# wizyoung/YOLOv3_TensorFlow

Measured on NVIDIA H100. Metric: images/sec, higher is better.
Workload: dtype f16

## Files before the change

yolov3_tensorflow_b200/csrc/common.cuh:

```cuda
#pragma once
#include <cuda.h>
#include <cuda_runtime.h>
#include <cuda_fp16.h>
#include <cuda_bf16.h>
#include <cuda_fp8.h>
#include <stdint.h>
#include <stdio.h>

#include "../../include/yolob200.h"

namespace yb {

void set_error(const char* fmt, ...);
int cuda_fail(cudaError_t e, const char* what, const char* file, int line);

#define YB_CUDA(call)                                                        \
  do {                                                                       \
    cudaError_t _e = (call);                                                 \
    if (_e != cudaSuccess) return yb::cuda_fail(_e, #call, __FILE__, __LINE__); \
  } while (0)

#define YB_REQUIRE(cond, ...)                \
  do {                                       \
    if (!(cond)) {                           \
// ... 105 lines not shown
}
__device__ __forceinline__ void mbar_wait(uint64_t* bar, uint32_t parity) {
  uint32_t spins = 0;
  while (!mbar_try_wait(bar, parity)) {
    if (++spins > (1u << 26)) __trap();
  }
}

__device__ __forceinline__ void tma_prefetch_desc(const CUtensorMap* m) {
  asm volatile("prefetch.tensormap [%0];" ::"l"(reinterpret_cast<uint64_t>(m)) : "memory");
}
__device__ __forceinline__ void tma_load_2d(void* dst, const CUtensorMap* m, uint64_t* bar, int c0, int c1) {
  asm volatile(
      "cp.async.bulk.tensor.2d.shared::cluster.global.tile.mbarrier::complete_tx::bytes [%0], [%1, {%3, %4}], [%2];"
      ::"r"(smem_u32(dst)), "l"(reinterpret_cast<uint64_t>(m)), "r"(smem_u32(bar)), "r"(c0), "r"(c1)
      : "memory");
}
__device__ __forceinline__ void tma_load_im2col_4d(void* dst, const CUtensorMap* m, uint64_t* bar, int c, int w,
                                                   int h, int n, uint16_t ow, uint16_t oh) {
  asm volatile(
      "cp.async.bulk.tensor.4d.shared::cluster.global.im2col.mbarrier::complete_tx::bytes"
      " [%0], [%1, {%3, %4, %5, %6}], [%2], {%7, %8};"
      ::"r"(smem_u32(dst)), "l"(reinterpret_cast<uint64_t>(m)), "r"(smem_u32(bar)), "r"(c), "r"(w), "r"(h),
      "r"(n), "h"(ow), "h"(oh)
      : "memory");
}

__device__ __forceinline__ void tma_store_2d(const CUtensorMap* m, const void* src, int c0, int c1) {
  asm volatile("cp.async.bulk.tensor.2d.global.shared::cta.bulk_group [%0, {%2, %3}], [%1];" ::"l"(
                   reinterpret_cast<uint64_t>(m)),
               "r"(smem_u32(src)), "r"(c0), "r"(c1)
               : "memory");
}
__device__ __forceinline__ void bulk_commit_group() { asm volatile("cp.async.bulk.commit_group;" ::: "memory"); }
template <int N>
__device__ __forceinline__ void bulk_wait_group_read() {
  asm volatile("cp.async.bulk.wait_group.read %0;" ::"n"(N) : "memory");
}
template <int N>
__device__ __forceinline__ void bulk_wait_group() {
  asm volatile("cp.async.bulk.wait_group %0;" ::"n"(N) : "memory");
}

__device__ __forceinline__ void stmatrix_x4(uint32_t saddr, uint32_t r0, uint32_t r1, uint32_t r2, uint32_t r3) {
  asm volatile("stmatrix.sync.aligned.m8n8.x4.shared.b16 [%0], {%1, %2, %3, %4};" ::"r"(saddr), "r"(r0), "r"(r1), "r"(r2),
               "r"(r3)
               : "memory");
}
__device__ __forceinline__ void ldmatrix_x4(uint32_t saddr, uint32_t& r0, uint32_t& r1, uint32_t& r2, uint32_t& r3) {
  asm volatile("ldmatrix.sync.aligned.m8n8.x4.shared.b16 {%0, %1, %2, %3}, [%4];"
               : "=r"(r0), "=r"(r1), "=r"(r2), "=r"(r3)
               : "r"(saddr)
               : "memory");
}

__device__ __forceinline__ uint32_t cluster_ctarank() {
  uint32_t r;
  asm volatile("mov.u32 %0, %%cluster_ctarank;" : "=r"(r));
  return r;
}
__device__ __forceinline__ void cluster_sync_all() {
  __syncwarp();
  asm volatile("barrier.cluster.arrive.release.aligned;" ::: "memory");
  asm volatile("barrier.cluster.wait.acquire.aligned;" ::: "memory");
}
__device__ __forceinline__ void mbar_arrive_remote(uint64_t* bar, uint32_t cta) {
// ... 58 lines not shown
```

yolov3_tensorflow_b200/csrc/conv.cuh:

```cuda
#pragma once
#include "common.cuh"
#include "decode.cuh"

namespace yb {

struct ConvParams {
  int M, P, Q;
  int cout;
  int cin;
  int ksize, stride, pad;
  int kh, kw;
  int scatter;
  int im2col;
  int consumers;
  int cluster;
  int cluster_n;
  int epi_reg;
  int pingpong;
  int ctas;
  int num_m_tiles, num_n_tiles;
  const float* scale;
  const float* shift;
  void* out;
  long out_ld;
// ... 7 lines not shown
  int res_smem;
  CUtensorMap tmR;
  int epi_tma;
  CUtensorMap tmO;
  int dtype;
  int block_n;
  int block_kb;
  int det_e;
};

struct ConvLaunch {
  CUtensorMap tmA, tmB;
  ConvParams p;
};

struct ConvRequest {
  yb_conv_desc d;
  int kh = 0, kw = 0, scatter = 0;
  bool stats = false;
  bool res = false;
  int det_e = 0;
  bool plan_rule = false;
};

int conv_select(const ConvRequest& r, ConvParams* p);
int conv_prepare(const ConvRequest& r, const void* x, const void* w_packed, const float* scale, const float* shift,
                 const void* res, void* out, float* stat_sum, float* stat_sqsum, ConvLaunch* l);
inline size_t dgrad_s2_class_offset(int c, int cin_pad, int k_cout) {
  static constexpr int first[4] = {0, 1, 3, 5};
  return (size_t)first[c] * cin_pad * k_cout;
}
int conv_prepare_dgrad_s2(const yb_conv_desc* fwd, const void* dz, int dz_ld, int k_cout, const void* w_dgrad_s2,
                          const void* res, int res_ld, void* dx, int dx_ld, ConvLaunch* l);
struct HaloMaps { CUtensorMap plane[4]; CUtensorMap w; CUtensorMap in3d; CUtensorMap res; };
struct HaloParams {
  int n, ho, wo;
  int tiles_x, tiles_y, num_tiles;
  int cout;
  int leaky;
  const float* scale;
  const float* shift;
  const void* res;
  long res_ld;
  void* out;
  long out_ld;
  const float* stem_w;
  const float* stem_scale;
  const float* stem_shift;
  int in_h, in_w;
  int out_e4m3;
  float out_inv_scale;
  int res_smem;
  int dtype;
  int cin, stride;
  int stem;
};
struct HaloRequest {
  yb_conv_desc d;
  bool res = false;
  bool out_e4m3 = false;
  bool stem = false;
};
struct HaloLaunch {
  HaloMaps maps;
  HaloParams p;
};
int halo_select(const HaloRequest& r, HaloParams* p);
// ... 33 lines not shown
```

yolov3_tensorflow_b200/csrc/conv_halo.cu:

```cuda
#include <cudaTypedefs.h>
#include <string.h>

#include <type_traits>

#include "common.cuh"
#include "conv.cuh"
#include "wgmma.cuh"

namespace yb {

int make_tmap_2d(CUtensorMap* tm, const void* base, int dtype, long rows, long cols, long ld, int box_rows, int box_cols,
                 int weights);
int make_tmap_image3d(CUtensorMap* tm, const float* base, int n, int h, int w, int box_f, int box_h);
int make_tmap_tiled4d(CUtensorMap* tm, const void* base, int dtype, int n, int h, int w, int c, long ld, int box_c,
                      int box_w, int box_h, int estride);

static constexpr int HT_H = 16, HT_W = 8;
static constexpr int HALO_THREADS = 384;
static constexpr int HALO_EPI_LD = 33;

template <int CIN, int COUT, int STRIDE, bool RES = false>
struct HaloCfg {
  static constexpr int ROWB = CIN * 2;
  static constexpr int NPLANE = STRIDE == 1 ? 1 : 4;
  static constexpr int ph(int p) { return STRIDE == 1 ? HT_H + 2 : ((p >> 1) == 0 ? HT_H + 1 : HT_H); }
  static constexpr int pw(int p) { return STRIDE == 1 ? HT_W + 2 : ((p & 1) == 0 ? HT_W + 1 : HT_W); }
  static constexpr int pbytes(int p) { return (ph(p) * pw(p) * ROWB + 1023) / 1024 * 1024; }
  static constexpr int poff(int p) { return p == 0 ? 0 : poff(p - 1) + pbytes(p - 1); }
  static constexpr int RES_OFF = poff(NPLANE - 1) + pbytes(NPLANE - 1);
  static constexpr int RES_BYTES = RES ? HT_H * HT_W * COUT * 2 : 0;
  static constexpr int STAGE_BYTES = RES_OFF + RES_BYTES;
  static constexpr int STAGE_TX = (STRIDE == 1 ? ph(0) * pw(0) * ROWB
                                               : (ph(0) * pw(0) + ph(1) * pw(1) + ph(2) * pw(2) + ph(3) * pw(3)) * ROWB) +
                                  RES_BYTES;
  static constexpr int B_TAP_BYTES = COUT * ROWB;
  static constexpr int B_BYTES = 9 * B_TAP_BYTES;
  static constexpr int EPI_BYTES = 2 * 64 * HALO_EPI_LD * 4;
  static constexpr int MISC_BYTES = 1024;
  static constexpr int BUDGET = 227 * 1024 - 1024 ;
  static constexpr int NST_RAW = (BUDGET - B_BYTES - EPI_BYTES - MISC_BYTES - 2 * COUT * 4) / STAGE_BYTES;
  static constexpr int NST = NST_RAW > 6 ? 6 : NST_RAW;
  static_assert(NST >= 1, "halo conv: configuration does not fit shared memory");
  static constexpr int SMEM_BYTES = 1024 + B_BYTES + NST * STAGE_BYTES + EPI_BYTES + MISC_BYTES + 2 * COUT * 4;
  static constexpr uint32_t SWIZZLE = ROWB;
  static constexpr int tap_plane(int r, int s) { return STRIDE == 1 ? 0 : (((r == 1) ? 2 : 0) | ((s == 1) ? 1 : 0)); }
  static constexpr int tap_dr(int r) { return STRIDE == 1 ? r : (r == 2 ? 1 : 0); }
  static constexpr int tap_ds(int s) { return STRIDE == 1 ? s : (s == 2 ? 1 : 0); }
};

struct StemCfg {
  static constexpr int SH = 2 * HT_H + 1, SW = 2 * HT_W + 1;
  static constexpr int NPX = SH * SW;
  static constexpr int NT16 = (NPX + 15) / 16;
  static constexpr int IN_ROWS = SH + 2;
  static constexpr int IN_ROWF = 60;
  static constexpr int IN_BYTES = (IN_ROWS * IN_ROWF * 4 + 127) / 128 * 128;
  static constexpr int NIN = 2;
};

__device__ __forceinline__ void tma_load_3d(void* dst, const CUtensorMap* m, uint64_t* bar, int c0, int c1, int c2) {
  asm volatile(
      "cp.async.bulk.tensor.3d.shared::cluster.global.tile.mbarrier::complete_tx::bytes [%0], [%1, {%3, %4, %5}], [%2];"
      ::"r"(smem_u32(dst)), "l"(reinterpret_cast<uint64_t>(m)), "r"(smem_u32(bar)), "r"(c0), "r"(c1), "r"(c2)
      : "memory");
}
__device__ __forceinline__ void mma16816_f16(float (&c)[4], const uint32_t (&a)[4], uint32_t b0, uint32_t b1, bool bf16) {
  if (bf16)
    asm volatile("mma.sync.aligned.m16n8k16.row.col.f32.bf16.bf16.f32 {%0,%1,%2,%3}, {%4,%5,%6,%7}, {%8,%9}, {%0,%1,%2,%3};"
                 : "+f"(c[0]), "+f"(c[1]), "+f"(c[2]), "+f"(c[3]) : "r"(a[0]), "r"(a[1]), "r"(a[2]), "r"(a[3]), "r"(b0), "r"(b1));
  else
    asm volatile("mma.sync.aligned.m16n8k16.row.col.f32.f16.f16.f32 {%0,%1,%2,%3}, {%4,%5,%6,%7}, {%8,%9}, {%0,%1,%2,%3};"
                 : "+f"(c[0]), "+f"(c[1]), "+f"(c[2]), "+f"(c[3]) : "r"(a[0]), "r"(a[1]), "r"(a[2]), "r"(a[3]), "r"(b0), "r"(b1));
}

__device__ __forceinline__ void tma_load_4d(void* dst, const CUtensorMap* m, uint64_t* bar, int c0, int c1, int c2, int c3) {
  asm volatile(
      "cp.async.bulk.tensor.4d.shared::cluster.global.tile.mbarrier::complete_tx::bytes [%0], [%1, {%3, %4, %5, %6}], [%2];"
      ::"r"(smem_u32(dst)), "l"(reinterpret_cast<uint64_t>(m)), "r"(smem_u32(bar)), "r"(c0), "r"(c1), "r"(c2), "r"(c3)
      : "memory");
}

template <typename T, int CIN, int COUT, int STRIDE, int STEMW = 0, typename TO = T, bool RES = false>
__global__ void __launch_bounds__(HALO_THREADS + 32 * STEMW, 1)
conv_halo_kernel(const __grid_constant__ HaloMaps maps, const __grid_constant__ HaloParams p) {
  using C = HaloCfg<CIN, COUT, STRIDE, RES>;
  static_assert(!RES || (CIN == 32 && COUT == 64 && STRIDE == 1 && STEMW == 0), "the residual box is Conv_3's");
  constexpr int PROD_WARP0 = HALO_THREADS / 32;
  static_assert(STEMW == 0 || (CIN == 32 && STRIDE == 2), "the fused stem feeds Conv_1 (32 -> 64, stride 2)");
  extern __shared__ uint8_t smem_raw[];
  uint8_t* smem = smem_raw + ((1024u - (smem_u32(smem_raw) & 1023u)) & 1023u);
  uint8_t* sB = smem;
  uint8_t* sA = smem + C::B_BYTES;
  float* sE = reinterpret_cast<float*>(sA + C::NST * C::STAGE_BYTES);
  uint64_t* bars = reinterpret_cast<uint64_t*>(reinterpret_cast<uint8_t*>(sE) + C::EPI_BYTES);
  uint64_t* full_bar = bars;
  uint64_t* empty_bar = bars + 8;
  uint64_t* b_bar = bars + 20;
  float* s_ss = reinterpret_cast<float*>(reinterpret_cast<uint8_t*>(sE) + C::EPI_BYTES + C::MISC_BYTES);
  uint64_t* in_full = bars + 24;
  uint64_t* in_empty = bars + 26;
  uint8_t* sIn = reinterpret_cast<uint8_t*>(s_ss + 2 * COUT);

  const int warp = threadIdx.x >> 5, lane = threadIdx.x & 31;

  if (warp == 0 && lane == 0) {
    if (STEMW == 0) {
#pragma unroll
      for (int i = 0; i < C::NPLANE; ++i) tma_prefetch_desc(&maps.plane[i]);
    }
    tma_prefetch_desc(&maps.w);
    if (RES) tma_prefetch_desc(&maps.res);
    for (int i = 0; i < C::NST; ++i) { mbar_init(&full_bar[i], STEMW > 0 ? STEMW : 1); mbar_init(&empty_bar[i], 8); }
    if (STEMW > 0) {
      tma_prefetch_desc(&maps.in3d);
      for (int i = 0; i < StemCfg::NIN; ++i) { mbar_init(&in_full[i], 1); mbar_init(&in_empty[i], STEMW); }
    }
    mbar_init(b_bar, 1);
    fence_barrier_init();
  }
  for (int c = threadIdx.x; c < COUT; c += blockDim.x) {
    s_ss[c] = c < p.cout ? __ldg(p.scale + c) : 0.f;
    s_ss[COUT + c] = c < p.cout ? __ldg(p.shift + c) : 0.f;
  }
  __syncthreads();

  if (warp == 0) {
    if (lane == 0) {
      mbar_arrive_expect_tx(b_bar, (uint32_t)C::B_BYTES);
#pragma unroll
      for (int t = 0; t < 9; ++t) tma_load_2d(sB + t * C::B_TAP_BYTES, &maps.w, b_bar, t * CIN, 0);
      int stage = 0;
      uint32_t phase = 0;
      if (STEMW > 0) {
        for (int tile = blockIdx.x; tile < p.num_tiles; tile += gridDim.x) {
          const int tx = tile % p.tiles_x;
          const int ty = (tile / p.tiles_x) % p.tiles_y;
          const int img = tile / (p.tiles_x * p.tiles_y);
          mbar_wait(&in_empty[stage], phase ^ 1);
          mbar_arrive_expect_tx(&in_full[stage], (uint32_t)(StemCfg::IN_ROWS * StemCfg::IN_ROWF * 4));
          tma_load_3d(sIn + stage * StemCfg::IN_BYTES, &maps.in3d, &in_full[stage], (2 * tx * HT_W - 2) * 3 - 2, 2 * ty * HT_H - 2, img);
          if (++stage == StemCfg::NIN) { stage = 0; phase ^= 1; }
        }
      }
      for (int tile = blockIdx.x; STEMW == 0 && tile < p.num_tiles; tile += gridDim.x) {
        const int tx = tile % p.tiles_x;
        const int ty = (tile / p.tiles_x) % p.tiles_y;
        const int img = tile / (p.tiles_x * p.tiles_y);
        const int h0 = ty * HT_H, w0 = tx * HT_W;
        mbar_wait(&empty_bar[stage], phase ^ 1);
        mbar_arrive_expect_tx(&full_bar[stage], (uint32_t)C::STAGE_TX);
        uint8_t* dst = sA + stage * C::STAGE_BYTES;
        if (STRIDE == 1) {
          tma_load_4d(dst, &maps.plane[0], &full_bar[stage], 0, w0 - 1, h0 - 1, img);
          if (RES) tma_load_4d(dst + C::RES_OFF, &maps.res, &full_bar[stage], 0, w0, h0, img);
        } else {
#pragma unroll
          for (int pl = 0; pl < 4; ++pl) {
            const int hs = 2 * h0 - ((pl >> 1) == 0 ? 1 : 0), ws = 2 * w0 - ((pl & 1) == 0 ? 1 : 0);
            tma_load_4d(dst + C::poff(pl), &maps.plane[pl], &full_bar[stage], 0, ws, hs, img);
          }
        }
        if (++stage == C::NST) { stage = 0; phase ^= 1; }
      }
    }
  } else if (warp >= 4 && warp < PROD_WARP0) {
    constexpr bool kBF16 = std::is_same<T, __nv_bfloat16>::value;
    const int cw = (warp - 4) >> 2;
    const int t = threadIdx.x & 127;
    const int bar_id = 1 + cw;
    float* stg = sE + cw * 64 * HALO_EPI_LD;
    const bool has_res = STEMW == 0 && p.res != nullptr;
    const int er = t >> 1, eh = t & 1;
    const uint32_t a_base = smem_u32(sA), b_base = smem_u32(sB);
    float acc[COUT / 2];
    mbar_wait(b_bar, 0);
    int stage = 0;
    uint32_t phase = 0;
    for (int tile = blockIdx.x; tile < p.num_tiles; tile += gridDim.x) {
      mbar_wait(&full_bar[stage], phase);
      const uint32_t st_base = a_base + stage * C::STAGE_BYTES;
      wgmma_fence_operand(acc);
      wgmma_fence();
#pragma unroll
      for (int r = 0; r < 3; ++r) {
#pragma unroll
        for (int s = 0; s < 3; ++s) {
          const int pl = C::tap_plane(r, s);
          const uint32_t a_tap = st_base + C::poff(pl) + ((8 * cw + C::tap_dr(r)) * C::pw(pl) + C::tap_ds(s)) * C::ROWB;
          const uint32_t b_tap = b_base + (r * 3 + s) * C::B_TAP_BYTES;
#pragma unroll
          for (int k = 0; k < CIN / 16; ++k)
            Wgmma<COUT, kBF16, 0, 0>::mma(acc, make_kmajor_desc(a_tap + k * 32, C::pw(pl) * C::ROWB, C::SWIZZLE),
                                          make_kmajor_desc(b_tap + k * 32, 8 * C::ROWB, C::SWIZZLE), (r | s | k) != 0);
        }
      }
      wgmma_commit();
      wgmma_fence_operand(acc);
      wgmma_wait<0>();
      wgmma_fence_operand(acc);
      const uint8_t* sres = sA + stage * C::STAGE_BYTES + C::RES_OFF;
      const int rel_stage = stage;
      if (!RES) {
        __syncwarp();
        if (lane == 0) mbar_arrive(&empty_bar[stage]);
      }
      if (++stage == C::NST) { stage = 0; phase ^= 1; }

      const int tx = tile % p.tiles_x;
      const int ty = (tile / p.tiles_x) % p.tiles_y;
      const int img = tile / (p.tiles_x * p.tiles_y);
      const int oh = ty * HT_H + 8 * cw + (er >> 3), ow = tx * HT_W + (er & 7);
      const bool ok = oh < p.ho && ow < p.wo;
      const long off = ((long)img * p.ho + oh) * p.wo + ow;
#pragma unroll 1
      for (int ch = 0; ch < COUT / 32; ++ch) {
        warpgroup_bar(bar_id);
        wgmma_stage_chunk<COUT>(acc, ch, stg, HALO_EPI_LD, t);
        warpgroup_bar(bar_id);
        if (!ok) continue;
        const int c0 = ch * 32 + eh * 16;
        const float* src = stg + er * HALO_EPI_LD + eh * 16;
        float v[16];
#pragma unroll
        for (int j = 0; j < 16; ++j) v[j] = fmaf(src[j], s_ss[c0 + j], s_ss[COUT + c0 + j]);
        if (p.leaky) {
#pragma unroll
          for (int j = 0; j < 16; ++j) v[j] = fmaxf(v[j], 0.1f * v[j]);
        }
        if (has_res) {
          const uint4* rp = reinterpret_cast<const uint4*>(static_cast<const T*>(p.res) + off * p.res_ld + c0);
          const int px = 64 * cw + er;
          const uint8_t* rrow = sres + px * 128;
#pragma unroll
          for (int j = 0; j < 2; ++j) {
            const uint4 u = RES ? *reinterpret_cast<const uint4*>(rrow + ((((c0 >> 3) + j) ^ (px & 7)) << 4)) : __ldg(rp + j);
            float2 f;
            f = Pack2<T>::unpack(u.x); v[8 * j + 0] += f.x; v[8 * j + 1] += f.y;
            f = Pack2<T>::unpack(u.y); v[8 * j + 2] += f.x; v[8 * j + 3] += f.y;
            f = Pack2<T>::unpack(u.z); v[8 * j + 4] += f.x; v[8 * j + 5] += f.y;
            f = Pack2<T>::unpack(u.w); v[8 * j + 6] += f.x; v[8 * j + 7] += f.y;
          }
        }
        if constexpr (std::is_same<TO, __nv_fp8_e4m3>::value) {
          *reinterpret_cast<uint4*>(static_cast<uint8_t*>(p.out) + off * p.out_ld + c0) = e4m3x16_pack(v, p.out_inv_scale);
          continue;
        }
        uint4* op = reinterpret_cast<uint4*>(static_cast<T*>(p.out) + off * p.out_ld + c0);
#pragma unroll
        for (int j = 0; j < 2; ++j) {
          uint4 pk;
          pk.x = Pack2<T>::pack(v[8 * j + 0], v[8 * j + 1]);
          pk.y = Pack2<T>::pack(v[8 * j + 2], v[8 * j + 3]);
          pk.z = Pack2<T>::pack(v[8 * j + 4], v[8 * j + 5]);
          pk.w = Pack2<T>::pack(v[8 * j + 6], v[8 * j + 7]);
          op[j] = pk;
        }
      }
      if (RES) {
        __syncwarp();
        if (lane == 0) mbar_arrive(&empty_bar[rel_stage]);
      }
    }
  } else if (STEMW > 0 && warp >= PROD_WARP0) {
    const int pw_id = warp - PROD_WARP0;
    const bool bf16 = std::is_same<T, __nv_bfloat16>::value;
    const int g = lane >> 2, q = lane & 3;
    uint32_t bfrag[4][2][2];
#pragma unroll
    for (int nt = 0; nt < 4; ++nt)
#pragma unroll
      for (int ks = 0; ks < 2; ++ks)
#pragma unroll
        for (int hb = 0; hb < 2; ++hb) {
          const int n = nt * 8 + g, k = ks * 16 + hb * 8 + 2 * q;
          const float w0 = k < 27 ? __ldg(p.stem_w + n * 27 + k) : 0.f;
          const float w1 = k + 1 < 27 ? __ldg(p.stem_w + n * 27 + k + 1) : 0.f;
          bfrag[nt][ks][hb] = Pack2<T>::pack(w0, w1);
        }
    float sc[4][2], sh[4][2];
#pragma unroll
    for (int nt = 0; nt < 4; ++nt)
#pragma unroll
      for (int j = 0; j < 2; ++j) {
        sc[nt][j] = __ldg(p.stem_scale + nt * 8 + 2 * q + j);
        sh[nt][j] = __ldg(p.stem_shift + nt * 8 + 2 * q + j);
      }
    int koff[2][2][2];
#pragma unroll
    for (int ks = 0; ks < 2; ++ks)
#pragma unroll
      for (int hb = 0; hb < 2; ++hb)
#pragma unroll
        for (int j = 0; j < 2; ++j) {
          const int k = ks * 16 + hb * 8 + 2 * q + j;
// ... 53 lines not shown
      auto store = [&](const M16& m) {
#pragma unroll
        for (int hr = 0; hr < 2; ++hr) {
          if (!m.live[hr]) continue;
          uint8_t* row = planes + m.poff + m.rho[hr] * 64 + q * 4;
          const int swz = (m.rho[hr] >> 1) & 3;
          if (m.inside[hr]) {
#pragma unroll
            for (int nt = 0; nt < 4; ++nt) {
              float v0 = fmaf(m.acc[nt][2 * hr], sc[nt][0], sh[nt][0]);
              float v1 = fmaf(m.acc[nt][2 * hr + 1], sc[nt][1], sh[nt][1]);
              v0 = fmaxf(v0, 0.1f * v0); v1 = fmaxf(v1, 0.1f * v1);
              *reinterpret_cast<uint32_t*>(row + ((nt ^ swz) << 4)) = Pack2<T>::pack(v0, v1);
            }
          } else {
#pragma unroll
            for (int nt = 0; nt < 4; ++nt) *reinterpret_cast<uint32_t*>(row + ((nt ^ swz) << 4)) = 0u;
          }
        }
      };
#pragma unroll 1
      for (int t = pw_id; t < StemCfg::NT16; t += STEMW) {
        M16 m0;
        gather(t, m0);
        multiply(m0);
        store(m0);
      }
      fence_proxy_async();
      __syncwarp();
      if (lane == 0) {
        mbar_arrive(&full_bar[stage]);
        mbar_arrive(&in_empty[in_stage]);
      }
      if (++in_stage == StemCfg::NIN) { in_stage = 0; in_phase ^= 1; }
      if (++stage == C::NST) { stage = 0; phase ^= 1; }
    }
  }
}

static constexpr int STEM_WARPS = 8;

template <typename T, int CIN, int COUT, int STRIDE, int STEMW = 0, typename TO = T, bool RES = false>
struct HaloKernel {
  static constexpr int THREADS = HALO_THREADS + 32 * STEMW;
  static constexpr int SMEM_BYTES =
      HaloCfg<CIN, COUT, STRIDE, RES>::SMEM_BYTES + (STEMW > 0 ? StemCfg::NIN * StemCfg::IN_BYTES : 0);
  static_assert(SMEM_BYTES <= 227 * 1024, "halo conv: configuration does not fit shared memory");
  static constexpr auto kernel = conv_halo_kernel<T, CIN, COUT, STRIDE, STEMW, TO, RES>;
};

static int no_halo_kernel(const HaloParams& p) {
  set_error("conv_halo: no kernel for dtype %d, cin=%d cout=%d stride=%d, fused stem %d, e4m3 output %d, residual box %d",
            p.dtype, p.cin, p.cout, p.stride, p.stem, p.out_e4m3, p.res_smem);
  return YB_ERR_UNSUPPORTED;
}

template <typename T, typename F>
static int halo_kernel_type(const HaloParams& p, F& f) {
  const int ci = p.cin, co = p.cout, s = p.stride;
  if (p.stem) {
    if (ci == 32 && co == 64 && s == 2 && !p.out_e4m3 && !p.res_smem) return f(HaloKernel<T, 32, 64, 2, STEM_WARPS>());
    return no_halo_kernel(p);
  }
  if (ci == 32 && co == 64 && s == 1) {
    if (!p.out_e4m3) return p.res_smem ? f(HaloKernel<T, 32, 64, 1, 0, T, true>()) : f(HaloKernel<T, 32, 64, 1>());
    if constexpr (std::is_same<T, __half>::value)
      return p.res_smem ? f(HaloKernel<T, 32, 64, 1, 0, __nv_fp8_e4m3, true>()) : f(HaloKernel<T, 32, 64, 1, 0, __nv_fp8_e4m3>());
    return no_halo_kernel(p);
  }
  if (p.out_e4m3 || p.res_smem) return no_halo_kernel(p);
  if (ci == 32 && co == 64 && s == 2) return f(HaloKernel<T, 32, 64, 2>());
  if (ci == 32 && co == 128 && s == 1) return f(HaloKernel<T, 32, 128, 1>());
  if (ci == 32 && co == 128 && s == 2) return f(HaloKernel<T, 32, 128, 2>());
  if (ci == 64 && co == 64 && s == 1) return f(HaloKernel<T, 64, 64, 1>());
  if (ci == 64 && co == 64 && s == 2) return f(HaloKernel<T, 64, 64, 2>());
  if (ci == 64 && co == 128 && s == 1) return f(HaloKernel<T, 64, 128, 1>());
  return no_halo_kernel(p);
}

// ... 45 lines not shown
  p->out_e4m3 = r.out_e4m3;
  p->res_smem = (r.res && !r.stem && d->cin == 32 && d->cout == 64 && d->stride == 1 &&
                 strcmp(opt("YB_CONV_RES"), "ldg") != 0) ? 1 : 0;
  p->dtype = d->dtype; p->cin = d->cin; p->stride = d->stride; p->stem = r.stem;
  return halo_kernel_for(*p, [](auto) -> int { return YB_OK; });
}

bool conv_halo_supported(const yb_conv_desc* d) {
  HaloParams p;
  return halo_select(HaloRequest{*d}, &p) == YB_OK;
}

int conv_halo_prepare(const HaloRequest& r, const void* x, const void* w_packed, const float* scale, const float* shift,
                      const void* res, void* out, const float* stem_w, const float* stem_scale, const float* stem_shift,
                      HaloLaunch* l) {
  HaloParams* p = &l->p;
  HaloMaps* maps = &l->maps;
  int rc = halo_select(r, p);
  if (rc) return rc;
  const yb_conv_desc* d = &r.d;
  YB_REQUIRE(x && w_packed && scale && shift && out, "conv_halo: null pointer");
  YB_REQUIRE(r.stem ? stem_w && stem_scale && stem_shift : !stem_w && !stem_scale && !stem_shift,
             "conv_halo: the stem's weights, scale and shift are given exactly when the request fuses the stem");
  YB_REQUIRE((res != nullptr) == r.res, "conv_halo: a residual pointer is given exactly when the request has a residual");
  YB_REQUIRE(((uintptr_t)x & 15) == 0 && ((uintptr_t)w_packed & 15) == 0 && ((uintptr_t)out & 15) == 0 && ((uintptr_t)res & 15) == 0,
             "conv_halo: pointers must be 16-byte aligned");
  memset(maps, 0, sizeof(*maps));
  p->scale = scale; p->shift = shift; p->res = res; p->out = out;
  p->stem_w = stem_w; p->stem_scale = stem_scale; p->stem_shift = stem_shift;
  if (p->res_smem) {
    rc = make_tmap_tiled4d(&maps->res, res, d->dtype, d->n, p->ho, p->wo, d->cout, d->res_ld, 64, HT_W, HT_H, 1);
    if (rc) return rc;
  }
  if (r.stem) {
    rc = make_tmap_image3d(&maps->in3d, static_cast<const float*>(x), d->n, d->h, d->w, StemCfg::IN_ROWF, StemCfg::IN_ROWS);
    if (rc) return rc;
  } else if (d->stride == 1) {
    rc = make_tmap_tiled4d(&maps->plane[0], x, d->dtype, d->n, d->h, d->w, d->cin, d->in_ld, d->cin, HT_W + 2, HT_H + 2, 1);
    if (rc) return rc;
  } else {
    for (int pl = 0; pl < 4; ++pl) {
      const int rows = (pl >> 1) == 0 ? HT_H + 1 : HT_H, cols = (pl & 1) == 0 ? HT_W + 1 : HT_W;
      rc = make_tmap_tiled4d(&maps->plane[pl], x, d->dtype, d->n, d->h, d->w, d->cin, d->in_ld, d->cin, 2 * cols - 1,
                             2 * rows - 1, 2);
      if (rc) return rc;
    }
  }
  const long K = 9L * d->cin;
  return make_tmap_2d(&maps->w, w_packed, d->dtype, yb_conv_cout_pad(d->cout), K, K, d->cout, d->cin, 1);
}

}

using namespace yb;

extern "C" int yb_conv3x3_halo_supported(const yb_conv_desc* d) { return d && conv_halo_supported(d) ? 1 : 0; }

extern "C" int yb_conv3x3_halo_fwd(const yb_conv_desc* d, const void* x, const void* w_packed, const float* scale,
                                   const float* shift, const void* res, void* out, void* stream) {
  if (!d) { set_error("conv_halo: null descriptor"); return YB_ERR_INVALID_ARGUMENT; }
  HaloRequest r{*d};
  r.res = res != nullptr;
  HaloLaunch l;
  int rc = conv_halo_prepare(r, x, w_packed, scale, shift, res, out, nullptr, nullptr, nullptr, &l);
  if (rc) return rc;
  return conv_halo_launch(l, static_cast<cudaStream_t>(stream));
// ... 14 lines not shown
```

yolov3_tensorflow_b200/csrc/conv_igemm.cu:

```cuda
#include <cudaTypedefs.h>
#include <math.h>
#include <stdlib.h>
#include <string.h>

#include <type_traits>

#include "common.cuh"
#include "conv.cuh"
#include "wgmma.cuh"

namespace yb {

static constexpr int WG_ROWS = 64;
static constexpr int RING_BYTES = 196 * 1024;
static constexpr int EPI_LD = 33;
static constexpr int EPI_FLOATS = WG_ROWS * EPI_LD;

template <int BN, int BKB, int NC, bool RES = false>
struct Cfg {
  static constexpr int BLOCK_M = WG_ROWS * NC;
  static constexpr int THREADS = 128 * (NC + 1);
  static constexpr int A_BYTES = BLOCK_M * BKB;
  static constexpr int B_BYTES = BN * BKB;
  static constexpr int STAGE_BYTES = A_BYTES + B_BYTES;
// ... 222 lines not shown
        }
      } else if (cany) {
        bool pass = false;
        float sc = 0.f;
        if (cok && v >= d.logit_lo) {
          sc = __fmul_rn(cconf, sigmoid_ref(v));
          pass = sc >= d.thr;
        }
        const unsigned m = __ballot_sync(0xffffffffu, pass);
        if (m != 0u) {
          const int c = e - 5;
          const unsigned mine = m & same;
          const int leader = pass ? __ffs(mine) - 1 : lane;
          int base = 0;
          if (pass && lane == leader) base = atomicAdd(d.cand_count + img * d.C + c, __popc(mine));
          base = __shfl_sync(0xffffffffu, base, leader);
          if (pass) {
            const long seg = ((long)img * d.C + c) * d.B;
            const int slot = base + __popc(mine & lt);
            d.cand_score[seg + slot] = sc;
            d.cand_idx[seg + slot] = box0 + a;
          }
        }
      }
      if (++e == E) { e = 0; ++a; }
    }
  }
}

template <typename T, int BN, int NH, bool RES>
__device__ __forceinline__ void epilogue_tma(const ConvParams& p, const float (&acc)[NH][BN / 2], const int row0,
                                             const int n0, const float4* ss4, uint8_t* slab, const uint32_t slab_h,
                                             const uint32_t slab_b, const int lane) {
  const int r = lane & 7, mi = lane >> 3;
  const uint32_t lane_off = (uint32_t)((r + 8 * (mi & 1)) * 128 + (((mi >> 1) ^ r) << 4));
  const float slope = p.leaky ? 0.1f : 1.f;
#pragma unroll
  for (int h = 0; h < NH; ++h) {
#pragma unroll
    for (int b = 0; b < BN / 64; ++b) {
      uint8_t* s = slab + h * slab_h + b * slab_b;
      const uint32_t sa = smem_u32(s) + lane_off;
      uint32_t pk[16];
#pragma unroll
      for (int q = 0; q < 4; ++q) {
        if constexpr (RES) ldmatrix_x4(sa ^ (q << 5), pk[4 * q], pk[4 * q + 1], pk[4 * q + 2], pk[4 * q + 3]);
#pragma unroll
        for (int ih = 0; ih < 2; ++ih) {
          const int j = 8 * b + 2 * q + ih;
          const float4 c = ss4[4 * j + (lane & 3)];
#pragma unroll
          for (int hh = 0; hh < 2; ++hh) {
            float v0 = fmaf(acc[h][4 * j + 2 * hh], c.x, c.z);
            float v1 = fmaf(acc[h][4 * j + 2 * hh + 1], c.y, c.w);
            v0 = fmaxf(v0, slope * v0);
            v1 = fmaxf(v1, slope * v1);
            uint32_t& w = pk[4 * q + 2 * ih + hh];
            if constexpr (RES) {
              const float2 f = Pack2<T>::unpack(w);
              v0 += f.x; v1 += f.y;
            }
            w = Pack2<T>::pack(v0, v1);
          }
        }
        if constexpr (RES) stmatrix_x4(sa ^ (q << 5), pk[4 * q], pk[4 * q + 1], pk[4 * q + 2], pk[4 * q + 3]);
      }
      if constexpr (!RES) {
        if (lane == 0) bulk_wait_group_read<0>();
        __syncwarp();
#pragma unroll
        for (int q = 0; q < 4; ++q) stmatrix_x4(sa ^ (q << 5), pk[4 * q], pk[4 * q + 1], pk[4 * q + 2], pk[4 * q + 3]);
      }
      fence_proxy_async();
      __syncwarp();
      if (lane == 0 && row0 + h * WG_ROWS < p.M && n0 + b * 64 < p.cout) {
        tma_store_2d(&p.tmO, s, n0 + b * 64, row0 + h * WG_ROWS);
        bulk_commit_group();
      }
    }
  }
}

static constexpr int MMA_TURN_BAR = 3;

template <typename T, int BN, int BKB, int NC, int DET_E = 0, bool PP = false, int CM = 0, int CN = 1, bool RES = false,
          bool TMA = false>
__global__ void __launch_bounds__(128 * (NC + 1), 1)
conv_igemm_kernel(const __grid_constant__ CUtensorMap tmA, const __grid_constant__ CUtensorMap tmB,
                  const __grid_constant__ ConvParams p) {
  static_assert(!PP || (NC == 2 && DET_E == 0), "ping-pong: two consumer warpgroups, no fused decode");
  static_assert(!RES || (PP && sizeof(T) == 2), "the shared-memory shortcut tile is a 16-bit ping-pong variant");
  static_assert(CM != 0 || CN == 1, "a run-time cluster shape is p.cluster x 1");
  static_assert(!TMA || (sizeof(T) == 2 && NC == 2 && DET_E == 0), "the TMA-store epilogue: 16-bit, 128-row tiles, no fused decode");
  constexpr int NH = PP ? 2 : 1;
  using C = Cfg<BN, BKB, NC, RES>;
  constexpr int BK = BKB / (int)sizeof(T);
  extern __shared__ uint8_t smem_raw[];
  uint8_t* smem = smem_raw + ((1024u - (smem_u32(smem_raw) & 1023u)) & 1023u);
  uint8_t* sA = smem;
  uint8_t* sB = smem + C::STAGES * C::A_BYTES;
  uint8_t* sR = smem + C::STAGES * C::STAGE_BYTES;
  float* s_epi = reinterpret_cast<float*>(sR + C::RES_BYTES);
  float* s_stat = s_epi + NC * EPI_FLOATS;
  float* s_ss = s_stat + NC * 2 * BN;
  uint64_t* full_bar = reinterpret_cast<uint64_t*>(s_ss + NC * 2 * BN);
  uint64_t* empty_bar = full_bar + 8;
  uint64_t* res_full = empty_bar + 8;
// ... 774 lines not shown
```

yolov3_tensorflow_b200/csrc/wgmma.cuh:

```cuda
#pragma once
#include <stdint.h>

namespace yb {

template <int N, bool BF16, int TA, int TB>
struct Wgmma;

template <int TA, int TB>
struct Wgmma<32, false, TA, TB> {
  static __device__ __forceinline__ void mma(float (&d)[16], uint64_t da, uint64_t db, int scale_d) {
    asm volatile(
        "{\n.reg .pred p;\nsetp.ne.b32 p, %18, 0;\n"
        "wgmma.mma_async.sync.aligned.m64n32k16.f32.f16.f16 {%0, %1, %2, %3, %4, %5, %6, %7, %8, %9, %10, %11, %12, %13, %14, %15}, %16, %17, p, 1, 1, %19, %20;\n}\n"
        : "+f"(d[0]), "+f"(d[1]), "+f"(d[2]), "+f"(d[3]), "+f"(d[4]), "+f"(d[5]), "+f"(d[6]), "+f"(d[7]), "+f"(d[8]), "+f"(d[9]), "+f"(d[10]), "+f"(d[11]), "+f"(d[12]), "+f"(d[13]), "+f"(d[14]), "+f"(d[15])
        : "l"(da), "l"(db), "r"(scale_d), "n"(TA), "n"(TB));
  }
};

template <int TA, int TB>
struct Wgmma<32, true, TA, TB> {
  static __device__ __forceinline__ void mma(float (&d)[16], uint64_t da, uint64_t db, int scale_d) {
    asm volatile(
        "{\n.reg .pred p;\nsetp.ne.b32 p, %18, 0;\n"
        "wgmma.mma_async.sync.aligned.m64n32k16.f32.bf16.bf16 {%0, %1, %2, %3, %4, %5, %6, %7, %8, %9, %10, %11, %12, %13, %14, %15}, %16, %17, p, 1, 1, %19, %20;\n}\n"
// ... 89 lines not shown
        "{\n.reg .pred p;\nsetp.ne.b32 p, %66, 0;\n"
        "wgmma.mma_async.sync.aligned.m64n128k32.f32.e4m3.e4m3 {%0, %1, %2, %3, %4, %5, %6, %7, %8, %9, %10, %11, %12, %13, %14, %15, %16, %17, %18, %19, %20, %21, %22, %23, %24, %25, %26, %27, %28, %29, %30, %31, %32, %33, %34, %35, %36, %37, %38, %39, %40, %41, %42, %43, %44, %45, %46, %47, %48, %49, %50, %51, %52, %53, %54, %55, %56, %57, %58, %59, %60, %61, %62, %63}, %64, %65, p, 1, 1;\n}\n"
        : "+f"(d[0]), "+f"(d[1]), "+f"(d[2]), "+f"(d[3]), "+f"(d[4]), "+f"(d[5]), "+f"(d[6]), "+f"(d[7]), "+f"(d[8]), "+f"(d[9]), "+f"(d[10]), "+f"(d[11]), "+f"(d[12]), "+f"(d[13]), "+f"(d[14]), "+f"(d[15]), "+f"(d[16]), "+f"(d[17]), "+f"(d[18]), "+f"(d[19]), "+f"(d[20]), "+f"(d[21]), "+f"(d[22]), "+f"(d[23]), "+f"(d[24]), "+f"(d[25]), "+f"(d[26]), "+f"(d[27]), "+f"(d[28]), "+f"(d[29]), "+f"(d[30]), "+f"(d[31]), "+f"(d[32]), "+f"(d[33]), "+f"(d[34]), "+f"(d[35]), "+f"(d[36]), "+f"(d[37]), "+f"(d[38]), "+f"(d[39]), "+f"(d[40]), "+f"(d[41]), "+f"(d[42]), "+f"(d[43]), "+f"(d[44]), "+f"(d[45]), "+f"(d[46]), "+f"(d[47]), "+f"(d[48]), "+f"(d[49]), "+f"(d[50]), "+f"(d[51]), "+f"(d[52]), "+f"(d[53]), "+f"(d[54]), "+f"(d[55]), "+f"(d[56]), "+f"(d[57]), "+f"(d[58]), "+f"(d[59]), "+f"(d[60]), "+f"(d[61]), "+f"(d[62]), "+f"(d[63])
        : "l"(da), "l"(db), "r"(scale_d));
  }
};

template <>
struct WgmmaE4M3<256> {
  static __device__ __forceinline__ void mma(float (&d)[128], uint64_t da, uint64_t db, int scale_d) {
    asm volatile(
        "{\n.reg .pred p;\nsetp.ne.b32 p, %130, 0;\n"
        "wgmma.mma_async.sync.aligned.m64n256k32.f32.e4m3.e4m3 {%0, %1, %2, %3, %4, %5, %6, %7, %8, %9, %10, %11, %12, %13, %14, %15, %16, %17, %18, %19, %20, %21, %22, %23, %24, %25, %26, %27, %28, %29, %30, %31, %32, %33, %34, %35, %36, %37, %38, %39, %40, %41, %42, %43, %44, %45, %46, %47, %48, %49, %50, %51, %52, %53, %54, %55, %56, %57, %58, %59, %60, %61, %62, %63, %64, %65, %66, %67, %68, %69, %70, %71, %72, %73, %74, %75, %76, %77, %78, %79, %80, %81, %82, %83, %84, %85, %86, %87, %88, %89, %90, %91, %92, %93, %94, %95, %96, %97, %98, %99, %100, %101, %102, %103, %104, %105, %106, %107, %108, %109, %110, %111, %112, %113, %114, %115, %116, %117, %118, %119, %120, %121, %122, %123, %124, %125, %126, %127}, %128, %129, p, 1, 1;\n}\n"
        : "+f"(d[0]), "+f"(d[1]), "+f"(d[2]), "+f"(d[3]), "+f"(d[4]), "+f"(d[5]), "+f"(d[6]), "+f"(d[7]), "+f"(d[8]), "+f"(d[9]), "+f"(d[10]), "+f"(d[11]), "+f"(d[12]), "+f"(d[13]), "+f"(d[14]), "+f"(d[15]), "+f"(d[16]), "+f"(d[17]), "+f"(d[18]), "+f"(d[19]), "+f"(d[20]), "+f"(d[21]), "+f"(d[22]), "+f"(d[23]), "+f"(d[24]), "+f"(d[25]), "+f"(d[26]), "+f"(d[27]), "+f"(d[28]), "+f"(d[29]), "+f"(d[30]), "+f"(d[31]), "+f"(d[32]), "+f"(d[33]), "+f"(d[34]), "+f"(d[35]), "+f"(d[36]), "+f"(d[37]), "+f"(d[38]), "+f"(d[39]), "+f"(d[40]), "+f"(d[41]), "+f"(d[42]), "+f"(d[43]), "+f"(d[44]), "+f"(d[45]), "+f"(d[46]), "+f"(d[47]), "+f"(d[48]), "+f"(d[49]), "+f"(d[50]), "+f"(d[51]), "+f"(d[52]), "+f"(d[53]), "+f"(d[54]), "+f"(d[55]), "+f"(d[56]), "+f"(d[57]), "+f"(d[58]), "+f"(d[59]), "+f"(d[60]), "+f"(d[61]), "+f"(d[62]), "+f"(d[63]), "+f"(d[64]), "+f"(d[65]), "+f"(d[66]), "+f"(d[67]), "+f"(d[68]), "+f"(d[69]), "+f"(d[70]), "+f"(d[71]), "+f"(d[72]), "+f"(d[73]), "+f"(d[74]), "+f"(d[75]), "+f"(d[76]), "+f"(d[77]), "+f"(d[78]), "+f"(d[79]), "+f"(d[80]), "+f"(d[81]), "+f"(d[82]), "+f"(d[83]), "+f"(d[84]), "+f"(d[85]), "+f"(d[86]), "+f"(d[87]), "+f"(d[88]), "+f"(d[89]), "+f"(d[90]), "+f"(d[91]), "+f"(d[92]), "+f"(d[93]), "+f"(d[94]), "+f"(d[95]), "+f"(d[96]), "+f"(d[97]), "+f"(d[98]), "+f"(d[99]), "+f"(d[100]), "+f"(d[101]), "+f"(d[102]), "+f"(d[103]), "+f"(d[104]), "+f"(d[105]), "+f"(d[106]), "+f"(d[107]), "+f"(d[108]), "+f"(d[109]), "+f"(d[110]), "+f"(d[111]), "+f"(d[112]), "+f"(d[113]), "+f"(d[114]), "+f"(d[115]), "+f"(d[116]), "+f"(d[117]), "+f"(d[118]), "+f"(d[119]), "+f"(d[120]), "+f"(d[121]), "+f"(d[122]), "+f"(d[123]), "+f"(d[124]), "+f"(d[125]), "+f"(d[126]), "+f"(d[127])
        : "l"(da), "l"(db), "r"(scale_d));
  }
};

template <int N>
__device__ __forceinline__ void wgmma_stage_chunk(const float (&acc)[N / 2], const int ch, float* dst, const int ld,
                                                  const int t) {
  const int r0 = 16 * (t >> 5) + ((t & 31) >> 2), c0 = 2 * (t & 3);
#pragma unroll
  for (int cc = 0; cc < N / 32; ++cc) {
    if (cc != ch) continue;
#pragma unroll
    for (int i = 0; i < 16; ++i) {
      const int row = r0 + 8 * ((i >> 1) & 1), col = 8 * (i >> 2) + c0 + (i & 1);
      dst[row * ld + col] = acc[cc * 16 + i];
    }
  }
}

}
```

Measured before the change: 6534.

## Route halo conv epilogue through swizzled smem slabs and 4D TMA stores

```diff
diff --git a/yolov3_tensorflow_b200/csrc/common.cuh b/yolov3_tensorflow_b200/csrc/common.cuh
--- a/yolov3_tensorflow_b200/csrc/common.cuh
+++ b/yolov3_tensorflow_b200/csrc/common.cuh
@@ -161,6 +161,12 @@
                "r"(smem_u32(src)), "r"(c0), "r"(c1)
                : "memory");
 }
+__device__ __forceinline__ void tma_store_4d(const CUtensorMap* m, const void* src, int c0, int c1, int c2, int c3) {
+  asm volatile("cp.async.bulk.tensor.4d.global.shared::cta.bulk_group [%0, {%2, %3, %4, %5}], [%1];" ::"l"(
+                   reinterpret_cast<uint64_t>(m)),
+               "r"(smem_u32(src)), "r"(c0), "r"(c1), "r"(c2), "r"(c3)
+               : "memory");
+}
 __device__ __forceinline__ void bulk_commit_group() { asm volatile("cp.async.bulk.commit_group;" ::: "memory"); }
 template <int N>
 __device__ __forceinline__ void bulk_wait_group_read() {
diff --git a/yolov3_tensorflow_b200/csrc/conv.cuh b/yolov3_tensorflow_b200/csrc/conv.cuh
--- a/yolov3_tensorflow_b200/csrc/conv.cuh
+++ b/yolov3_tensorflow_b200/csrc/conv.cuh
@@ -63,7 +63,7 @@
 }
 int conv_prepare_dgrad_s2(const yb_conv_desc* fwd, const void* dz, int dz_ld, int k_cout, const void* w_dgrad_s2,
                           const void* res, int res_ld, void* dx, int dx_ld, ConvLaunch* l);
-struct HaloMaps { CUtensorMap plane[4]; CUtensorMap w; CUtensorMap in3d; CUtensorMap res; };
+struct HaloMaps { CUtensorMap plane[4]; CUtensorMap w; CUtensorMap in3d; CUtensorMap res; CUtensorMap out; };
 struct HaloParams {
   int n, ho, wo;
   int tiles_x, tiles_y, num_tiles;
diff --git a/yolov3_tensorflow_b200/csrc/conv_halo.cu b/yolov3_tensorflow_b200/csrc/conv_halo.cu
--- a/yolov3_tensorflow_b200/csrc/conv_halo.cu
+++ b/yolov3_tensorflow_b200/csrc/conv_halo.cu
@@ -19,7 +19,18 @@
 static constexpr int HALO_THREADS = 384;
 static constexpr int HALO_EPI_LD = 33;
 
-template <int CIN, int COUT, int STRIDE, bool RES = false>
+struct StemCfg {
+  static constexpr int SH = 2 * HT_H + 1, SW = 2 * HT_W + 1;
+  static constexpr int NPX = SH * SW;
+  static constexpr int NT16 = (NPX + 15) / 16;
+  static constexpr int IN_ROWS = SH + 2;
+  static constexpr int IN_ROWF = 60;
+  static constexpr int IN_BYTES = (IN_ROWS * IN_ROWF * 4 + 127) / 128 * 128;
+  static constexpr int NST = 2;
+  static constexpr int NIN_MAX = 8;
+};
+
+template <int CIN, int COUT, int STRIDE, bool RES = false, bool TMA = false, int STEMW = 0>
 struct HaloCfg {
   static constexpr int ROWB = CIN * 2;
   static constexpr int NPLANE = STRIDE == 1 ? 1 : 4;
@@ -35,27 +46,22 @@
                                   RES_BYTES;
   static constexpr int B_TAP_BYTES = COUT * ROWB;
   static constexpr int B_BYTES = 9 * B_TAP_BYTES;
-  static constexpr int EPI_BYTES = 2 * 64 * HALO_EPI_LD * 4;
+  static constexpr int EPI_BYTES = (TMA && RES) ? 0 : ((TMA && STEMW > 0) ? 8 * 2048 : 2 * 64 * HALO_EPI_LD * 4);
   static constexpr int MISC_BYTES = 1024;
+  static constexpr int SS_BYTES = 4 * COUT * 4;
   static constexpr int BUDGET = 227 * 1024 - 1024 ;
-  static constexpr int NST_RAW = (BUDGET - B_BYTES - EPI_BYTES - MISC_BYTES - 2 * COUT * 4) / STAGE_BYTES;
-  static constexpr int NST = NST_RAW > 6 ? 6 : NST_RAW;
-  static_assert(NST >= 1, "halo conv: configuration does not fit shared memory");
-  static constexpr int SMEM_BYTES = 1024 + B_BYTES + NST * STAGE_BYTES + EPI_BYTES + MISC_BYTES + 2 * COUT * 4;
+  static constexpr int FIXED = B_BYTES + EPI_BYTES + MISC_BYTES + SS_BYTES;
+  static constexpr int NST_RAW = (BUDGET - FIXED) / STAGE_BYTES;
+  static constexpr int NST = STEMW > 0 ? StemCfg::NST : (NST_RAW > 6 ? 6 : NST_RAW);
+  static_assert(NST >= 1 && NST <= 8, "halo conv: configuration does not fit shared memory");
+  static constexpr int NIN_RAW = STEMW > 0 ? (BUDGET - FIXED - NST * STAGE_BYTES) / StemCfg::IN_BYTES : 0;
+  static constexpr int NIN = NIN_RAW > StemCfg::NIN_MAX ? StemCfg::NIN_MAX : NIN_RAW;
+  static_assert(STEMW == 0 || NIN >= 2, "halo conv: the fused stem's image ring does not fit shared memory");
+  static constexpr int SMEM_BYTES = 1024 + FIXED + NST * STAGE_BYTES + NIN * StemCfg::IN_BYTES;
   static constexpr uint32_t SWIZZLE = ROWB;
   static constexpr int tap_plane(int r, int s) { return STRIDE == 1 ? 0 : (((r == 1) ? 2 : 0) | ((s == 1) ? 1 : 0)); }
   static constexpr int tap_dr(int r) { return STRIDE == 1 ? r : (r == 2 ? 1 : 0); }
   static constexpr int tap_ds(int s) { return STRIDE == 1 ? s : (s == 2 ? 1 : 0); }
-};
-
-struct StemCfg {
-  static constexpr int SH = 2 * HT_H + 1, SW = 2 * HT_W + 1;
-  static constexpr int NPX = SH * SW;
-  static constexpr int NT16 = (NPX + 15) / 16;
-  static constexpr int IN_ROWS = SH + 2;
-  static constexpr int IN_ROWF = 60;
-  static constexpr int IN_BYTES = (IN_ROWS * IN_ROWF * 4 + 127) / 128 * 128;
-  static constexpr int NIN = 2;
 };
 
 __device__ __forceinline__ void tma_load_3d(void* dst, const CUtensorMap* m, uint64_t* bar, int c0, int c1, int c2) {
@@ -83,10 +89,12 @@
 template <typename T, int CIN, int COUT, int STRIDE, int STEMW = 0, typename TO = T, bool RES = false>
 __global__ void __launch_bounds__(HALO_THREADS + 32 * STEMW, 1)
 conv_halo_kernel(const __grid_constant__ HaloMaps maps, const __grid_constant__ HaloParams p) {
-  using C = HaloCfg<CIN, COUT, STRIDE, RES>;
+  constexpr bool kTMA = !std::is_same<TO, __nv_fp8_e4m3>::value;
+  using C = HaloCfg<CIN, COUT, STRIDE, RES, kTMA, STEMW>;
   static_assert(!RES || (CIN == 32 && COUT == 64 && STRIDE == 1 && STEMW == 0), "the residual box is Conv_3's");
   constexpr int PROD_WARP0 = HALO_THREADS / 32;
   static_assert(STEMW == 0 || (CIN == 32 && STRIDE == 2), "the fused stem feeds Conv_1 (32 -> 64, stride 2)");
+  static_assert(STEMW == 0 || kTMA, "the fused stem's Conv_1 has a 16-bit output");
   extern __shared__ uint8_t smem_raw[];
   uint8_t* smem = smem_raw + ((1024u - (smem_u32(smem_raw) & 1023u)) & 1023u);
   uint8_t* sB = smem;
@@ -96,10 +104,11 @@
   uint64_t* full_bar = bars;
   uint64_t* empty_bar = bars + 8;
   uint64_t* b_bar = bars + 20;
+  uint64_t* in_full = bars + 32;
+  uint64_t* in_empty = bars + 48;
   float* s_ss = reinterpret_cast<float*>(reinterpret_cast<uint8_t*>(sE) + C::EPI_BYTES + C::MISC_BYTES);
-  uint64_t* in_full = bars + 24;
-  uint64_t* in_empty = bars + 26;
-  uint8_t* sIn = reinterpret_cast<uint8_t*>(s_ss + 2 * COUT);
+  float* s_ss4 = s_ss + 2 * COUT;
+  uint8_t* sIn = reinterpret_cast<uint8_t*>(s_ss + 4 * COUT);
 
   const int warp = threadIdx.x >> 5, lane = threadIdx.x & 31;
 
@@ -110,17 +119,21 @@
     }
     tma_prefetch_desc(&maps.w);
     if (RES) tma_prefetch_desc(&maps.res);
+    if (kTMA) tma_prefetch_desc(&maps.out);
     for (int i = 0; i < C::NST; ++i) { mbar_init(&full_bar[i], STEMW > 0 ? STEMW : 1); mbar_init(&empty_bar[i], 8); }
     if (STEMW > 0) {
       tma_prefetch_desc(&maps.in3d);
-      for (int i = 0; i < StemCfg::NIN; ++i) { mbar_init(&in_full[i], 1); mbar_init(&in_empty[i], STEMW); }
+      for (int i = 0; i < C::NIN; ++i) { mbar_init(&in_full[i], 1); mbar_init(&in_empty[i], STEMW); }
     }
     mbar_init(b_bar, 1);
     fence_barrier_init();
   }
   for (int c = threadIdx.x; c < COUT; c += blockDim.x) {
-    s_ss[c] = c < p.cout ? __ldg(p.scale + c) : 0.f;
-    s_ss[COUT + c] = c < p.cout ? __ldg(p.shift + c) : 0.f;
+    const float sc = c < p.cout ? __ldg(p.scale + c) : 0.f, sh = c < p.cout ? __ldg(p.shift + c) : 0.f;
+    s_ss[c] = sc;
+    s_ss[COUT + c] = sh;
+    s_ss4[(c >> 1) * 4 + (c & 1)] = sc;
+    s_ss4[(c >> 1) * 4 + 2 + (c & 1)] = sh;
   }
   __syncthreads();
 
@@ -139,7 +152,7 @@
           mbar_wait(&in_empty[stage], phase ^ 1);
           mbar_arrive_expect_tx(&in_full[stage], (uint32_t)(StemCfg::IN_ROWS * StemCfg::IN_ROWF * 4));
           tma_load_3d(sIn + stage * StemCfg::IN_BYTES, &maps.in3d, &in_full[stage], (2 * tx * HT_W - 2) * 3 - 2, 2 * ty * HT_H - 2, img);
-          if (++stage == StemCfg::NIN) { stage = 0; phase ^= 1; }
+          if (++stage == C::NIN) { stage = 0; phase ^= 1; }
         }
       }
       for (int tile = blockIdx.x; STEMW == 0 && tile < p.num_tiles; tile += gridDim.x) {
@@ -171,6 +184,7 @@
     float* stg = sE + cw * 64 * HALO_EPI_LD;
     const bool has_res = STEMW == 0 && p.res != nullptr;
     const int er = t >> 1, eh = t & 1;
+    const float slope = p.leaky ? 0.1f : 1.f;
     const uint32_t a_base = smem_u32(sA), b_base = smem_u32(sB);
     float acc[COUT / 2];
     mbar_wait(b_bar, 0);
@@ -209,6 +223,26 @@
       const int tx = tile % p.tiles_x;
       const int ty = (tile / p.tiles_x) % p.tiles_y;
       const int img = tile / (p.tiles_x * p.tiles_y);
+      if constexpr (kTMA) {
+        if (RES || !has_res) {
+          const int wq = (warp - 4) & 3, oh0 = ty * HT_H + 8 * cw + 2 * wq;
+          uint8_t* slab = RES ? sA + rel_stage * C::STAGE_BYTES + C::RES_OFF + (64 * cw + 16 * wq) * 128
+                              : reinterpret_cast<uint8_t*>(sE) + (warp - 4) * 2048;
+#pragma unroll
+          for (int b = 0; b < COUT / 64; ++b) {
+            epi_box_to_slab<T, COUT, RES>(acc, b, reinterpret_cast<const float4*>(s_ss4), slab, slope, lane);
+            if (lane == 0 && oh0 < p.ho) {
+              tma_store_4d(&maps.out, slab, 64 * b, tx * HT_W, oh0, img);
+              bulk_commit_group();
+            }
+          }
+          if (RES && lane == 0) {
+            bulk_wait_group_read<0>();
+            mbar_arrive(&empty_bar[rel_stage]);
+          }
+          continue;
+        }
+      }
       const int oh = ty * HT_H + 8 * cw + (er >> 3), ow = tx * HT_W + (er & 7);
       const bool ok = oh < p.ho && ow < p.wo;
       const long off = ((long)img * p.ho + oh) * p.wo + ow;
@@ -260,6 +294,9 @@
         __syncwarp();
         if (lane == 0) mbar_arrive(&empty_bar[rel_stage]);
       }
+    }
+    if constexpr (kTMA) {
+      if (lane == 0) bulk_wait_group<0>();
     }
   } else if (STEMW > 0 && warp >= PROD_WARP0) {
     const int pw_id = warp - PROD_WARP0;
@@ -379,19 +416,19 @@
         mbar_arrive(&full_bar[stage]);
         mbar_arrive(&in_empty[in_stage]);
       }
-      if (++in_stage == StemCfg::NIN) { in_stage = 0; in_phase ^= 1; }
+      if (++in_stage == C::NIN) { in_stage = 0; in_phase ^= 1; }
       if (++stage == C::NST) { stage = 0; phase ^= 1; }
     }
   }
 }
 
-static constexpr int STEM_WARPS = 8;
+static constexpr int STEM_WARPS = 12;
 
 template <typename T, int CIN, int COUT, int STRIDE, int STEMW = 0, typename TO = T, bool RES = false>
 struct HaloKernel {
   static constexpr int THREADS = HALO_THREADS + 32 * STEMW;
   static constexpr int SMEM_BYTES =
-      HaloCfg<CIN, COUT, STRIDE, RES>::SMEM_BYTES + (STEMW > 0 ? StemCfg::NIN * StemCfg::IN_BYTES : 0);
+      HaloCfg<CIN, COUT, STRIDE, RES, !std::is_same<TO, __nv_fp8_e4m3>::value, STEMW>::SMEM_BYTES;
   static_assert(SMEM_BYTES <= 227 * 1024, "halo conv: configuration does not fit shared memory");
   static constexpr auto kernel = conv_halo_kernel<T, CIN, COUT, STRIDE, STEMW, TO, RES>;
 };
@@ -503,6 +540,10 @@
     rc = make_tmap_tiled4d(&maps->res, res, d->dtype, d->n, p->ho, p->wo, d->cout, d->res_ld, 64, HT_W, HT_H, 1);
     if (rc) return rc;
   }
+  if (!p->out_e4m3) {
+    rc = make_tmap_tiled4d(&maps->out, out, d->dtype, d->n, p->ho, p->wo, d->cout, d->out_ld, 64, HT_W, 2, 1);
+    if (rc) return rc;
+  }
   if (r.stem) {
     rc = make_tmap_image3d(&maps->in3d, static_cast<const float*>(x), d->n, d->h, d->w, StemCfg::IN_ROWF, StemCfg::IN_ROWS);
     if (rc) return rc;
diff --git a/yolov3_tensorflow_b200/csrc/conv_igemm.cu b/yolov3_tensorflow_b200/csrc/conv_igemm.cu
--- a/yolov3_tensorflow_b200/csrc/conv_igemm.cu
+++ b/yolov3_tensorflow_b200/csrc/conv_igemm.cu
@@ -278,47 +278,13 @@
 __device__ __forceinline__ void epilogue_tma(const ConvParams& p, const float (&acc)[NH][BN / 2], const int row0,
                                              const int n0, const float4* ss4, uint8_t* slab, const uint32_t slab_h,
                                              const uint32_t slab_b, const int lane) {
-  const int r = lane & 7, mi = lane >> 3;
-  const uint32_t lane_off = (uint32_t)((r + 8 * (mi & 1)) * 128 + (((mi >> 1) ^ r) << 4));
   const float slope = p.leaky ? 0.1f : 1.f;
 #pragma unroll
   for (int h = 0; h < NH; ++h) {
 #pragma unroll
     for (int b = 0; b < BN / 64; ++b) {
       uint8_t* s = slab + h * slab_h + b * slab_b;
-      const uint32_t sa = smem_u32(s) + lane_off;
-      uint32_t pk[16];
-#pragma unroll
-      for (int q = 0; q < 4; ++q) {
-        if constexpr (RES) ldmatrix_x4(sa ^ (q << 5), pk[4 * q], pk[4 * q + 1], pk[4 * q + 2], pk[4 * q + 3]);
-#pragma unroll
-        for (int ih = 0; ih < 2; ++ih) {
-          const int j = 8 * b + 2 * q + ih;
-          const float4 c = ss4[4 * j + (lane & 3)];
-#pragma unroll
-          for (int hh = 0; hh < 2; ++hh) {
-            float v0 = fmaf(acc[h][4 * j + 2 * hh], c.x, c.z);
-            float v1 = fmaf(acc[h][4 * j + 2 * hh + 1], c.y, c.w);
-            v0 = fmaxf(v0, slope * v0);
-            v1 = fmaxf(v1, slope * v1);
-            uint32_t& w = pk[4 * q + 2 * ih + hh];
-            if constexpr (RES) {
-              const float2 f = Pack2<T>::unpack(w);
-              v0 += f.x; v1 += f.y;
-            }
-            w = Pack2<T>::pack(v0, v1);
-          }
-        }
-        if constexpr (RES) stmatrix_x4(sa ^ (q << 5), pk[4 * q], pk[4 * q + 1], pk[4 * q + 2], pk[4 * q + 3]);
-      }
-      if constexpr (!RES) {
-        if (lane == 0) bulk_wait_group_read<0>();
-        __syncwarp();
-#pragma unroll
-        for (int q = 0; q < 4; ++q) stmatrix_x4(sa ^ (q << 5), pk[4 * q], pk[4 * q + 1], pk[4 * q + 2], pk[4 * q + 3]);
-      }
-      fence_proxy_async();
-      __syncwarp();
+      epi_box_to_slab<T, BN, RES>(acc[h], b, ss4, s, slope, lane);
       if (lane == 0 && row0 + h * WG_ROWS < p.M && n0 + b * 64 < p.cout) {
         tma_store_2d(&p.tmO, s, n0 + b * 64, row0 + h * WG_ROWS);
         bulk_commit_group();
diff --git a/yolov3_tensorflow_b200/csrc/wgmma.cuh b/yolov3_tensorflow_b200/csrc/wgmma.cuh
--- a/yolov3_tensorflow_b200/csrc/wgmma.cuh
+++ b/yolov3_tensorflow_b200/csrc/wgmma.cuh
@@ -145,4 +145,43 @@
   }
 }
 
+template <typename T, int N, bool RES>
+__device__ __forceinline__ void epi_box_to_slab(const float (&acc)[N / 2], const int b, const float4* ss4, uint8_t* slab,
+                                                const float slope, const int lane) {
+  const int r = lane & 7, mi = lane >> 3;
+  const uint32_t sa = smem_u32(slab) + (uint32_t)((r + 8 * (mi & 1)) * 128 + (((mi >> 1) ^ r) << 4));
+  uint32_t pk[16];
+#pragma unroll
+  for (int q = 0; q < 4; ++q) {
+    if constexpr (RES) ldmatrix_x4(sa ^ (q << 5), pk[4 * q], pk[4 * q + 1], pk[4 * q + 2], pk[4 * q + 3]);
+#pragma unroll
+    for (int ih = 0; ih < 2; ++ih) {
+      const int j = 8 * b + 2 * q + ih;
+      const float4 c = ss4[4 * j + (lane & 3)];
+#pragma unroll
+      for (int hh = 0; hh < 2; ++hh) {
+        float v0 = fmaf(acc[4 * j + 2 * hh], c.x, c.z);
+        float v1 = fmaf(acc[4 * j + 2 * hh + 1], c.y, c.w);
+        v0 = fmaxf(v0, slope * v0);
+        v1 = fmaxf(v1, slope * v1);
+        uint32_t& w = pk[4 * q + 2 * ih + hh];
+        if constexpr (RES) {
+          const float2 f = Pack2<T>::unpack(w);
+          v0 += f.x; v1 += f.y;
+        }
+        w = Pack2<T>::pack(v0, v1);
+      }
+    }
+    if constexpr (RES) stmatrix_x4(sa ^ (q << 5), pk[4 * q], pk[4 * q + 1], pk[4 * q + 2], pk[4 * q + 3]);
+  }
+  if constexpr (!RES) {
+    if (lane == 0) bulk_wait_group_read<0>();
+    __syncwarp();
+#pragma unroll
+    for (int q = 0; q < 4; ++q) stmatrix_x4(sa ^ (q << 5), pk[4 * q], pk[4 * q + 1], pk[4 * q + 2], pk[4 * q + 3]);
+  }
+  fence_proxy_async();
+  __syncwarp();
 }
+
+}
```

New measurement: 6752, median of 6. +3.3%, better.
